# lukifer23/Matrix0

Measured on NVIDIA B200. Metric: MCTS sims/sec, batched self-play, ResNet-24 (BASELINE configs[3]), higher is better.
Workload: dtype fp16

## Files before the change

matrix0_b200/csrc/nn_attention_tc.cu:

```cuda
#include "nn.cuh"
#include <cuda_fp16.h>
#include <cstdlib>

namespace m0 {

template <bool FP16>
__device__ __forceinline__ void mma16816(float (&d)[4], const uint32_t (&a)[4], const uint32_t (&b)[2]) {
  if (FP16) {
    asm volatile("mma.sync.aligned.m16n8k16.row.col.f32.f16.f16.f32 {%0,%1,%2,%3}, {%4,%5,%6,%7}, {%8,%9}, {%0,%1,%2,%3};"
                 : "+f"(d[0]), "+f"(d[1]), "+f"(d[2]), "+f"(d[3])
                 : "r"(a[0]), "r"(a[1]), "r"(a[2]), "r"(a[3]), "r"(b[0]), "r"(b[1]));
  } else {
    asm volatile("mma.sync.aligned.m16n8k16.row.col.f32.bf16.bf16.f32 {%0,%1,%2,%3}, {%4,%5,%6,%7}, {%8,%9}, {%0,%1,%2,%3};"
                 : "+f"(d[0]), "+f"(d[1]), "+f"(d[2]), "+f"(d[3])
                 : "r"(a[0]), "r"(a[1]), "r"(a[2]), "r"(a[3]), "r"(b[0]), "r"(b[1]));
  }
}
template <bool FP16>
__device__ __forceinline__ uint32_t pack2(float lo, float hi) {
  if (FP16) {
    __half2 h = __floats2half2_rn(lo, hi);
    return *reinterpret_cast<uint32_t*>(&h);
  }
  __nv_bfloat162 h = __floats2bfloat162_rn(lo, hi);
// ... 277 lines not shown
  if (staged) {
    const int smem = 2 * 64 * BIAS_LD * (int)sizeof(float) + 8 * ATT_STAGE_BYTES;
    static unsigned long long granted = 0;
    int dev = 0;
    cudaGetDevice(&dev);
    if (dev >= 64 || !((granted >> dev) & 1ull)) {
      cudaError_t e = cudaFuncSetAttribute(attention_tc_staged_kernel<true>, cudaFuncAttributeMaxDynamicSharedMemorySize, smem);
      if (e == cudaSuccess) e = cudaFuncSetAttribute(attention_tc_staged_kernel<false>, cudaFuncAttributeMaxDynamicSharedMemorySize, smem);
      if (e != cudaSuccess) { m0_set_error("attention_tc: cannot reserve %d bytes of shared memory (%s)", smem, cudaGetErrorString(e)); return M0_ERR_CUDA; }
      if (dev < 64) granted |= 1ull << dev;
    }
    dim3 grid(heads, (B + 8 * bpw - 1) / (8 * bpw));
    if (nn_half_format()) attention_tc_staged_kernel<true><<<grid, 256, smem, s>>>((const uint16_t*)qkv_half, rel_bias, (uint16_t*)out_half, B, C, mix, bpw);
    else attention_tc_staged_kernel<false><<<grid, 256, smem, s>>>((const uint16_t*)qkv_half, rel_bias, (uint16_t*)out_half, B, C, mix, bpw);
    return m0_check_launch("attention_tc_staged");
  }
  const int per_block = 8 * ATT_BOARDS_PER_WARP;
  dim3 grid(heads, (B + per_block - 1) / per_block);
  if (nn_half_format()) attention_tc_kernel<true><<<grid, 256, 0, s>>>((const uint16_t*)qkv_half, rel_bias, (uint16_t*)out_half, B, C, mix);
  else attention_tc_kernel<false><<<grid, 256, 0, s>>>((const uint16_t*)qkv_half, rel_bias, (uint16_t*)out_half, B, C, mix);
  return m0_check_launch("attention_tc");
}

}
```

matrix0_b200/csrc/nn_tc_kernels.cu:

```cuda
#include "net_host.cuh"
#include "tc_gemm.cuh"
#include "tc_conv_pair.cuh"
#include <new>
#include <stdlib.h>
#include <string.h>
#include <stdio.h>
#include <string>
#include <utility>
#include <vector>

using namespace m0;

namespace m0 {
int nn_se_apply_gn(const __nv_bfloat16* conv_out, const float* gate, float* x, const float* gamma, const float* beta, __nv_bfloat16* a_out, int B,
                   int C, int act, cudaStream_t s);
int nn_planes_to_nhwc_half(const float* planes, __nv_bfloat16* out, int B, int P, cudaStream_t s);
int nn_se_hidden(const float* part, int splits, long long split_stride, const float* b1, __nv_bfloat16* hidden, int B, int hid, int ld, int act,
                 cudaStream_t s);
int nn_gn_act_res(const float* x, const float* gamma, const float* beta, const float* residual, long long residual_bstride, float* out,
                  __nv_bfloat16* out_half, int B, int C, int act, cudaStream_t s);
int nn_attention_tc(const void* qkv_half, const float* rel_bias, void* out_half, int B, int C, int heads, float mix, cudaStream_t s);
int nn_se_tail(const float* part, int splits, long long split_stride, int ld, const float* b1, const float* w2t, const float* b2, float* gate, int B,
               int C, int hid, int act, cudaStream_t s);
int nn_value_tail(const float* gate, const float* h, const float* w3, const float* b3, float* values, int B, int C, cudaStream_t s);
int nn_se_gate(const float* pool, const float* w1t, const float* b1, const float* w2t, const float* b2, float* gate, int B, int C, int hid, int act,
               cudaStream_t s);
}

namespace m0 {
__global__ void transpose_f32_kernel(const float* __restrict__ in, float* __restrict__ out, int rows, int cols) {
  int i = blockIdx.x * blockDim.x + threadIdx.x;
  if (i >= rows * cols) return;
  int r = i / cols, c = i % cols;
  out[c * rows + r] = in[i];
}
__global__ void se_fold_kernel(const float* __restrict__ conv_w, const float* __restrict__ w1, float* __restrict__ out, int C, int hid) {
  const int K = 12 * C;
  const int i = blockIdx.x * blockDim.x + threadIdx.x;
  if (i >= hid * K) return;
  const int u = i / K, k = i - u * K;
  const int ci = k % C, j = (k / C) % 6, hb = k / (6 * C);
  unsigned plus = 0, minus = 0;
  switch (j) {
    case 0: plus = 0x1FF; break;
// ... 84 lines not shown
struct TcWeight {
  __nv_bfloat16* w = nullptr;
  CUtensorMap map;
  CUtensorMap map_pair;
  bool pair = false;
  int n = 0, k = 0, n_part = 0, cluster = 1;
  int n_launch = 0;
};

int pick_cluster(int n_part) {
  static int forced = -1;
  if (forced < 0) {
    const char* e = getenv("M0_TC_CLUSTER");
    forced = e ? atoi(e) : 0;
  }
  int cs = forced > 0 ? forced : 2;
  while (cs > 1 && ((n_part / cs) % 8 != 0 || n_part % cs != 0)) cs >>= 1;
  return cs;
}

struct TcBlock {
  TcWeight conv1, conv2, qkv, proj;
  TcWeight se_fold, se_w2;
};

struct TcState {
  int sm_count = 148;
  int max_smem = 0;
  size_t smem_pair[9] = {0, 0, 0, 0, 0, 0, 0, 0, 0};
  size_t smem_gemm = 0;
  TcWeight pst, inter;
  std::vector<TcBlock> blocks;
  float *pool = nullptr, *se_hid = nullptr, *se_gate = nullptr;
  std::vector<float*> se_w1t, se_w2t;
  bool se_fused = false;
  int hid_pad = 0;
  __nv_bfloat16 *prims = nullptr, *se_hid_h = nullptr;
  float* se_part = nullptr;
  int se_splits = 1;
  size_t se_rows = 0;
  CUtensorMap prims_mat, se_hid_mat;
  __nv_bfloat16* planes_h = nullptr;
  __nv_bfloat16* qkv_h = nullptr;
  bool heads_tc = false;
  TcWeight pol_conv, pol_fc1, pol_fc2, val_conv1, val_conv2, val_fc1, val_fc2, val_gate;
  bool val_tail_tc = false;
  int pol_rank_pad = 0;
  __nv_bfloat16 *ph_h = nullptr, *pf_h = nullptr, *vh_h = nullptr;
  __nv_bfloat16 *vf1_h = nullptr, *vf2_h = nullptr;
  CUtensorMap ph_mat, pf_mat, vh_conv_mat, vh_fc_mat, vf1_mat, vf2_mat;
  CUtensorMap planes_conv;
  TcWeight stem;
  int cap = 0;
  __nv_bfloat16 *a1 = nullptr, *a2 = nullptr;
  CUtensorMap a1_conv, a2_conv, a1_mat, a2_mat;
  CUtensorMap a1_convp, a2_convp, planes_convp;
  CUtensorMap x_io;
  const void* x_ptr = nullptr;
  CUtensorMap qkv_out, t2f_out;
  CUtensorMap a1_out, a2_out, t1_out, t2h_out;
  const void *t1_ptr = nullptr, *t2_ptr = nullptr;
  int out_rows = 0;
  std::vector<void*> allocs;
};

// ... 300 lines not shown
  if (st->se_gate) cudaFree(st->se_gate);
  if (st->planes_h) cudaFree(st->planes_h);
  if (st->qkv_h) cudaFree(st->qkv_h);
  if (st->ph_h) cudaFree(st->ph_h);
  if (st->pf_h) cudaFree(st->pf_h);
  if (st->vh_h) cudaFree(st->vh_h);
  if (st->vf1_h) cudaFree(st->vf1_h);
  if (st->vf2_h) cudaFree(st->vf2_h);
  st->vf1_h = st->vf2_h = nullptr;
  if (st->prims) cudaFree(st->prims);
  if (st->se_hid_h) cudaFree(st->se_hid_h);
  if (st->se_part) cudaFree(st->se_part);
  st->se_part = nullptr;
  st->prims = st->se_hid_h = nullptr;
  st->qkv_h = st->ph_h = st->pf_h = st->vh_h = nullptr;
  st->a1 = st->a2 = nullptr;
  st->pool = st->se_hid = st->se_gate = nullptr;
  st->planes_h = nullptr;
  st->cap = 0;
  M0_CUDA_TRY(cudaMalloc((void**)&st->pool, (size_t)need * 2 * C * 4));
  M0_CUDA_TRY(cudaMalloc((void**)&st->se_hid, (size_t)need * (n->cfg.se_hidden > 0 ? n->cfg.se_hidden : 1) * 4));
  M0_CUDA_TRY(cudaMalloc((void**)&st->se_gate, (size_t)need * C * 4));
  M0_CUDA_TRY(cudaMalloc((void**)&st->planes_h, (size_t)need * 64 * 64 * 2));
  M0_CUDA_TRY(cudaMalloc((void**)&st->qkv_h, (size_t)need * 64 * 3 * C * 2));
  if (st->heads_tc) {
    const size_t rp = (size_t)st->pol_rank_pad;
    M0_CUDA_TRY(cudaMalloc((void**)&st->ph_h, (size_t)need * 4096 * 2));
    M0_CUDA_TRY(cudaMalloc((void**)&st->pf_h, (size_t)need * rp * 2));
    M0_CUDA_TRY(cudaMalloc((void**)&st->vh_h, (size_t)need * 8192 * 2));
    M0_CUDA_TRY(cudaMemset(st->pf_h, 0, (size_t)need * rp * 2));
    TRY(make_map_2d(&st->ph_mat, st->ph_h, (uint64_t)need, 4096, 128));
    TRY(make_map_2d(&st->pf_mat, st->pf_h, (uint64_t)need, rp, 128));
    TRY(make_map_2d(&st->vh_conv_mat, st->vh_h, (uint64_t)need * 64, 128, 128));
    TRY(make_map_2d(&st->vh_fc_mat, st->vh_h, (uint64_t)need, 8192, 128));
    if (st->val_tail_tc) {
      M0_CUDA_TRY(cudaMalloc((void**)&st->vf1_h, (size_t)need * 2 * C * 2));
      M0_CUDA_TRY(cudaMalloc((void**)&st->vf2_h, (size_t)need * C * 2));
      TRY(make_map_2d(&st->vf1_mat, st->vf1_h, (uint64_t)need, 2 * C, 128));
      TRY(make_map_2d(&st->vf2_mat, st->vf2_h, (uint64_t)need, C, 128));
    }
  }
  if (st->se_fused && n->cfg.se) {
    const size_t rows = ((size_t)need + 127) / 128 * 128;
    M0_CUDA_TRY(cudaMalloc((void**)&st->prims, rows * 12 * C * 2));
    M0_CUDA_TRY(cudaMalloc((void**)&st->se_hid_h, rows * st->hid_pad * 2));
    M0_CUDA_TRY(cudaMemset(st->prims, 0, rows * 12 * C * 2));
    M0_CUDA_TRY(cudaMemset(st->se_hid_h, 0, rows * st->hid_pad * 2));
// ... 77 lines not shown
      if ((rc = m0_check_cuda(cudaMemsetAsync(w2p, 0, (size_t)ps_pad * rp * 4, s), "memset")) != M0_OK) break;
      if ((rc = m0_check_cuda(cudaMemcpy2DAsync(w2p, (size_t)rp * 4, n->w.pol_fc2_w, (size_t)r * 4, (size_t)r * 4, c.policy_size,
                                                cudaMemcpyDeviceToDevice, s), "pad pol_fc2")) != M0_OK) break;
      if ((rc = make_weight(st, &st->pol_conv, n->w.pol_conv_w, 64, C, 64, s)) != M0_OK) break;
      if ((rc = make_weight(st, &st->pol_fc1, n->w.pol_fc1_w, r, 4096, r, s)) != M0_OK) break;
      if ((rc = make_weight(st, &st->pol_fc2, w2p, ps_pad, rp, 320, s)) != M0_OK) break;
      if ((rc = make_weight(st, &st->val_conv1, n->w.val_conv1_w, 128, C, 128, s)) != M0_OK) break;
      if ((rc = make_weight(st, &st->val_conv2, n->w.val_conv2_w, 128, 128, 128, s)) != M0_OK) break;
      const int fc1_launch = n_part_for(C) % 32 == 0 ? C : slice_width_for(C, C);
      if ((rc = make_weight(st, &st->val_fc1, n->w.val_fc1_w, 2 * C, 8192, fc1_launch, s)) != M0_OK) break;
      if (env_int("M0_TC_VALUE_TAIL", 1)) {
        if ((rc = make_weight(st, &st->val_fc2, n->w.val_fc2_w, C, 2 * C, slice_width_for(C, C), s)) != M0_OK) break;
        if ((rc = make_weight(st, &st->val_gate, n->w.val_gate_w, C, C, slice_width_for(C, C), s)) != M0_OK) break;
        st->val_tail_tc = true;
      }
      st->heads_tc = true;
    }
    if (c.chess_features) {
      if (c.piece_square_tables && (rc = make_weight(st, &st->pst, n->w.pst_w, C, C, env_int("M0_TC_SLICE_PROJ", 1) ? slice_width_for(C, C) : C, s)) != M0_OK) break;
      if ((rc = make_weight(st, &st->inter, n->w.inter_w, C, 9 * C, C, s, 9)) != M0_OK) break;
    }
    st->hid_pad = (c.se_hidden + 63) / 64 * 64;
    st->se_fused = env_int("M0_TC_FUSE_SE", 1) != 0 && pair_ok(C) && (!c.se || c.se_hidden <= 256);
    st->blocks.resize(c.blocks);
    for (int i = 0; i < c.blocks && rc == M0_OK; ++i) {
      const m0_block_weights& b = n->w.blocks[i];
      if ((rc = make_weight(st, &st->blocks[i].conv1, b.conv1_w, C, 9 * C, C, s, 9)) != M0_OK) break;
      if ((rc = make_weight(st, &st->blocks[i].conv2, b.conv2_w, C, 9 * C, C, s, 9)) != M0_OK) break;
      if (st->se_fused && c.se) {
        const int hid = c.se_hidden, hid16 = (hid + 15) / 16 * 16, K = 12 * C, hp = st->hid_pad;
        float *fold = nullptr, *w2p = nullptr;
        if ((rc = m0_check_cuda(cudaMalloc((void**)&fold, (size_t)hid16 * K * 4), "cudaMalloc se_fold")) != M0_OK) break;
        st->allocs.push_back(fold);
        if ((rc = m0_check_cuda(cudaMemsetAsync(fold, 0, (size_t)hid16 * K * 4, s), "memset se_fold")) != M0_OK) break;
        if ((rc = m0_check_cuda(cudaMalloc((void**)&w2p, (size_t)C * hp * 4), "cudaMalloc se_w2")) != M0_OK) break;
        st->allocs.push_back(w2p);
        se_fold_kernel<<<(hid * K + 255) / 256, 256, 0, s>>>(b.conv2_w, b.se_w1, fold, C, hid);
        pad_cols_kernel<float><<<(C * hp + 255) / 256, 256, 0, s>>>(b.se_w2, w2p, C, hid, hp);
        if ((rc = m0_check_launch("se_fold")) != M0_OK) break;
        if ((rc = make_weight(st, &st->blocks[i].se_fold, fold, hid16, K, hid16, s)) != M0_OK) break;
        if ((rc = make_weight(st, &st->blocks[i].se_w2, w2p, C, hp, C, s)) != M0_OK) break;
      }
      if (b.has_attention) {
        if ((rc = make_weight(st, &st->blocks[i].qkv, b.att_qkv_w, 3 * C, C, slice_width_for(3 * C, C), s)) != M0_OK) break;
        if ((rc = make_weight(st, &st->blocks[i].proj, b.att_proj_w, C, C, env_int("M0_TC_SLICE_PROJ", 1) ? slice_width_for(C, C) : C, s)) != M0_OK) break;
      }
    }
  } while (0);
  if (rc != M0_OK) {
    for (void* p : st->allocs) cudaFree(p);
    delete st;
    return rc;
  }
  all->st[fmt] = st;
  return M0_OK;
}

void tc_net_release(::m0_net* n) {
  TcStates* all = (TcStates*)n->tc;
  if (!all) return;
  for (int f = 0; f < 2; ++f) {
    TcState* st = all->st[f];
    if (!st) continue;
    for (void* p : st->allocs) cudaFree(p);
    if (st->a1) cudaFree(st->a1);
    if (st->a2) cudaFree(st->a2);
    if (st->pool) cudaFree(st->pool);
// ... 9 lines not shown
    if (st->prims) cudaFree(st->prims);
    if (st->se_hid_h) cudaFree(st->se_hid_h);
    if (st->se_part) cudaFree(st->se_part);
    delete st;
  }
  delete all;
  n->tc = nullptr;
}

int tc_net_forward(::m0_net* n, const float* planes, int B, float* logits, float* values, cudaStream_t s) {
  TcState* st = ((TcStates*)n->tc)->st[nn_half_format()];
  TRY(net_ws_reserve(n, B));
  TRY(tc_reserve(n, st, B));
  const m0_net_config& c = n->cfg;
  const m0_net_weights& w = n->w;
  const int C = c.channels, M = B * 64, act = c.activation;
  const float* none = nullptr;
  if (st->t1_ptr != n->t1 || st->t2_ptr != n->t2 || st->x_ptr != n->x || st->out_rows != M) {
    TRY(make_map_out(&st->a1_out, st->a1, (uint64_t)M, C, false));
    TRY(make_map_out(&st->a2_out, st->a2, (uint64_t)M, C, false));
    TRY(make_map_out(&st->t1_out, n->t1, (uint64_t)M, C, true));
    TRY(make_map_out(&st->t2h_out, n->t2, (uint64_t)M, C, false));
    TRY(make_map_out(&st->t2f_out, n->t2, (uint64_t)M, C, true));
    TRY(make_map_out(&st->qkv_out, st->qkv_h, (uint64_t)M, 3 * (uint64_t)C, false));
    TRY(make_map_out(&st->x_io, n->x, (uint64_t)M, C, true, true));
    st->x_ptr = n->x;
    st->t1_ptr = n->t1;
    st->t2_ptr = n->t2;
    st->out_rows = M;
  }
  PROF("planes_to_nhwc_half", nn_planes_to_nhwc_half(planes, st->planes_h, B, c.planes, s));
  PROF("conv_other", conv3x3(st, st->planes_conv, st->planes_convp, st->stem, B, 64, n->t1, nullptr, ACT_NONE, s, nullptr, nullptr, nullptr, nullptr, &st->t1_out));
  if (c.chess_features) {
    PROF("gn_act_res", nn_gn_act_res(n->t1, w.stem_gn_w, w.stem_gn_b, w.pos_enc, 0, n->x, st->a1, B, C, act, s));
    float* cur = n->x;
    if (c.piece_square_tables) {
      PROF("gemm_pst", gemm_rows64(st, st->a1_mat, st->pst, B, C, n->t1, nullptr, C, s, &st->t1_out));
      PROF("gn_act_res", nn_gn_act_res(n->t1, w.pst_gn_w, w.pst_gn_b, n->x, (long long)64 * C, n->t2, st->a1, B, C, act, s));
      cur = n->t2;
    }
    PROF("conv_other", conv3x3(st, st->a1_conv, st->a1_convp, st->inter, B, C, n->t1, nullptr, ACT_NONE, s, nullptr, nullptr, nullptr, nullptr, &st->t1_out));
    PROF("gn_act_res", nn_gn_act_res(n->t1, w.inter_gn_w, w.inter_gn_b, cur, (long long)64 * C, n->x, nullptr, B, C, act, s));
  } else {
    PROF("groupnorm_f32", nn_groupnorm_f32(n->t1, w.stem_gn_w, w.stem_gn_b, nullptr, 0, n->x, B, C, act, s));
  }
  if (c.blocks > 0) PROF("se_apply_gn", nn_se_apply_gn(nullptr, nullptr, n->x, w.blocks[0].gn1_w, w.blocks[0].gn1_b, st->a1, B, C, act, s));
  int att_seen = 0;
// ... 37 lines not shown
      se_done:;
      }
      ConvFusion f2;
      f2.resid_x = n->x;
      f2.gate = c.se ? st->se_gate : nullptr;
      f2.x_map = &st->x_io;
      PROF("conv2+se+res+gn", conv3x3(st, st->a2_conv, st->a2_convp, tb.conv2, B, C, nullptr, next_a, act, s, fuse_next ? w.blocks[i + 1].gn1_w : nullptr,
                                      fuse_next ? w.blocks[i + 1].gn1_b : nullptr, nullptr, &f2, next_a ? &st->a1_out : nullptr));
    } else {
      PROF("conv1+gn", conv3x3(st, st->a1_conv, st->a1_convp, tb.conv1, B, C, nullptr, st->a2, act, s, b.gn2_w, b.gn2_b, nullptr, nullptr, &st->a2_out));
      __nv_bfloat16* t2h = reinterpret_cast<__nv_bfloat16*>(n->t2);
      PROF("conv2+pool", conv3x3(st, st->a2_conv, st->a2_convp, tb.conv2, B, C, nullptr, t2h, ACT_NONE, s, nullptr, nullptr, c.se ? st->pool : nullptr, nullptr,
                                 &st->t2h_out));
      const float* gate = nullptr;
      if (c.se) {
        PROF("se_gate", nn_se_gate(st->pool, st->se_w1t[i], b.se_b1, st->se_w2t[i], b.se_b2, st->se_gate, B, C, c.se_hidden, act, s));
        gate = st->se_gate;
      }
      PROF("se_apply_gn", nn_se_apply_gn(t2h, gate, n->x, fuse_next ? w.blocks[i + 1].gn1_w : nullptr, fuse_next ? w.blocks[i + 1].gn1_b : nullptr,
                                         next_a, B, C, act, s));
    }
    if (run_att) {
      const float* rb = c.attention_relbias ? b.att_rel_bias : nullptr;
      if (tc_att) {
        PROF("gemm_qkv", gemm_rows64(st, st->a1_mat, tb.qkv, B, C, nullptr, st->qkv_h, 3 * C, s, &st->qkv_out));
        PROF("attention_tc", nn_attention_tc(st->qkv_h, rb, st->a2, B, C, c.attention_heads, c.attention_unmasked_mix, s));
      } else {
        PROF("gemm_qkv", gemm_rows64(st, st->a1_mat, tb.qkv, B, C, n->qkv, nullptr, 3 * C, s));
        PROF("attention_f32", nn_attention_f32(n->qkv, rb, n->t1, B, C, c.attention_heads, c.attention_unmasked_mix, s));
        PROF("f32_to_bf16", nn_f32_to_bf16(n->t1, st->a2, (size_t)M * C, s));
      }
      static int proj_f32 = -1;
      if (proj_f32 < 0) proj_f32 = env_int("M0_TC_PROJ_F32", 0);
      const bool fused_ln = C % 32 == 0 && C <= 320;
      const bool proj_half = fused_ln && !proj_f32;
      if (proj_half) PROF("gemm_proj", gemm_rows64(st, st->a2_mat, tb.proj, B, C, nullptr, reinterpret_cast<__nv_bfloat16*>(n->t2), C, s, &st->t2h_out));
      else PROF("gemm_proj", gemm_rows64(st, st->a2_mat, tb.proj, B, C, n->t2, nullptr, C, s, &st->t2f_out));
      if (fused_ln) {
        heads_input_ready = last && st->heads_tc;
        PROF("ln_res_gn", nn_ln_res_gn(n->t2, proj_half ? 1 : 0, n->x, b.att_ln_w, b.att_ln_b, last ? nullptr : w.blocks[i + 1].gn1_w,
                                       last ? nullptr : w.blocks[i + 1].gn1_b, (last && !st->heads_tc) ? nullptr : st->a1, B, C, act, s));
      } else {
        PROF("layernorm_residual_f32", nn_layernorm_residual_f32(n->t2, n->x, b.att_ln_w, b.att_ln_b, n->x, M, C, s));
        if (!last) PROF("se_apply_gn", nn_se_apply_gn(nullptr, nullptr, n->x, w.blocks[i + 1].gn1_w, w.blocks[i + 1].gn1_b, st->a1, B, C, act, s));
      }
    }
  }
// ... 116 lines not shown
```

matrix0_b200/csrc/tc_gemm.cuh:

```cuda
#pragma once
#include <cuda.h>
#include <cuda_bf16.h>
#include <cuda_fp16.h>
#include "nn.cuh"

namespace m0 {
namespace tc {

static constexpr int BM = 128;
static constexpr int BK = 64;
static constexpr int A_TILE_BYTES = BM * BK * 2;
static constexpr int NUM_THREADS = 320;

__device__ __forceinline__ uint32_t smem_u32(const void* p) { return (uint32_t)__cvta_generic_to_shared(p); }

__device__ __forceinline__ void mbar_init(uint64_t* bar, uint32_t count) {
  asm volatile("mbarrier.init.shared::cta.b64 [%0], %1;" ::"r"(smem_u32(bar)), "r"(count) : "memory");
}
__device__ __forceinline__ void mbar_expect_tx(uint64_t* bar, uint32_t bytes) {
  asm volatile("mbarrier.arrive.expect_tx.shared::cta.b64 _, [%0], %1;" ::"r"(smem_u32(bar)), "r"(bytes) : "memory");
}
__device__ __forceinline__ void mbar_arrive(uint64_t* bar) {
  asm volatile("mbarrier.arrive.shared::cta.b64 _, [%0];" ::"r"(smem_u32(bar)) : "memory");
}
__device__ __forceinline__ void mbar_wait(uint64_t* bar, uint32_t parity) {
  asm volatile(
      "{\n\t"
      ".reg .pred p;\n\t"
      "WAIT_%=:\n\t"
      "mbarrier.try_wait.parity.shared::cta.b64 p, [%0], %1;\n\t"
      "@p bra DONE_%=;\n\t"
      "bra WAIT_%=;\n\t"
      "DONE_%=:\n\t"
      "}\n" ::"r"(smem_u32(bar)), "r"(parity)
      : "memory");
}
__device__ __forceinline__ void fence_barrier_init() { asm volatile("fence.mbarrier_init.release.cluster;" ::: "memory"); }
__device__ __forceinline__ void fence_proxy_async() { asm volatile("fence.proxy.async.shared::cta;" ::: "memory"); }

__device__ __forceinline__ void tma_prefetch_desc(const CUtensorMap* m) {
  asm volatile("prefetch.tensormap [%0];" ::"l"(reinterpret_cast<uint64_t>(m)) : "memory");
}
__device__ __forceinline__ void tma_load_2d(void* dst, const CUtensorMap* map, uint64_t* bar, int c0, int c1) {
  asm volatile("cp.async.bulk.tensor.2d.shared::cluster.global.mbarrier::complete_tx::bytes [%0], [%1, {%3, %4}], [%2];" ::"r"(smem_u32(dst)),
               "l"(reinterpret_cast<uint64_t>(map)), "r"(smem_u32(bar)), "r"(c0), "r"(c1)
               : "memory");
}
__device__ __forceinline__ void tma_load_4d(void* dst, const CUtensorMap* map, uint64_t* bar, int c0, int c1, int c2, int c3) {
  asm volatile("cp.async.bulk.tensor.4d.shared::cluster.global.mbarrier::complete_tx::bytes [%0], [%1, {%3, %4, %5, %6}], [%2];" ::"r"(
                   smem_u32(dst)),
               "l"(reinterpret_cast<uint64_t>(map)), "r"(smem_u32(bar)), "r"(c0), "r"(c1), "r"(c2), "r"(c3)
               : "memory");
}

__device__ __forceinline__ void tma_load_2d_mcast(void* dst, const CUtensorMap* map, uint64_t* bar, int c0, int c1, uint16_t cta_mask) {
  asm volatile(
      "cp.async.bulk.tensor.2d.shared::cluster.global.mbarrier::complete_tx::bytes.multicast::cluster [%0], [%1, {%3, %4}], [%2], %5;" ::"r"(
          smem_u32(dst)),
      "l"(reinterpret_cast<uint64_t>(map)), "r"(smem_u32(bar)), "r"(c0), "r"(c1), "h"(cta_mask)
      : "memory");
}
__device__ __forceinline__ bool elect_one() {
  uint32_t pred;
  asm volatile(
      "{\n\t"
      ".reg .pred P;\n\t"
      "elect.sync _|P, 0xFFFFFFFF;\n\t"
      "selp.u32 %0, 1, 0, P;\n\t"
      "}\n"
      : "=r"(pred));
  return pred != 0;
}
__device__ __forceinline__ uint32_t cluster_ctarank() {
  uint32_t r;
  asm volatile("mov.u32 %0, %%cluster_ctarank;" : "=r"(r));
  return r;
}
__device__ __forceinline__ void cluster_sync_all() {
  asm volatile("barrier.cluster.arrive.release.aligned;" ::: "memory");
  asm volatile("barrier.cluster.wait.acquire.aligned;" ::: "memory");
}

__device__ __forceinline__ void tmem_alloc(uint32_t* dst_smem, uint32_t cols) {
  asm volatile("tcgen05.alloc.cta_group::1.sync.aligned.shared::cta.b32 [%0], %1;" ::"r"(smem_u32(dst_smem)), "r"(cols) : "memory");
}
__device__ __forceinline__ void tmem_relinquish() { asm volatile("tcgen05.relinquish_alloc_permit.cta_group::1.sync.aligned;" ::: "memory"); }
__device__ __forceinline__ void tmem_dealloc(uint32_t addr, uint32_t cols) {
  asm volatile("tcgen05.dealloc.cta_group::1.sync.aligned.b32 %0, %1;" ::"r"(addr), "r"(cols) : "memory");
}
__device__ __forceinline__ void tc_fence_before() { asm volatile("tcgen05.fence::before_thread_sync;" ::: "memory"); }
__device__ __forceinline__ void tc_fence_after() { asm volatile("tcgen05.fence::after_thread_sync;" ::: "memory"); }

__device__ __forceinline__ void umma_bf16(uint32_t tmem_d, uint64_t desc_a, uint64_t desc_b, uint32_t idesc, uint32_t accumulate) {
  asm volatile(
      "{\n\t"
      ".reg .pred p;\n\t"
      "setp.ne.b32 p, %4, 0;\n\t"
      "tcgen05.mma.cta_group::1.kind::f16 [%0], %1, %2, %3, p;\n\t"
      "}\n" ::"r"(tmem_d),
      "l"(desc_a), "l"(desc_b), "r"(idesc), "r"(accumulate)
      : "memory");
}
__device__ __forceinline__ void umma_commit(uint64_t* bar) {
  asm volatile("tcgen05.commit.cta_group::1.mbarrier::arrive::one.shared::cluster.b64 [%0];" ::"r"(smem_u32(bar)) : "memory");
}
__device__ __forceinline__ void umma_commit_mcast(uint64_t* bar, uint16_t cta_mask) {
  asm volatile("tcgen05.commit.cta_group::1.mbarrier::arrive::one.shared::cluster.multicast::cluster.b64 [%0], %1;" ::"r"(smem_u32(bar)),
               "h"(cta_mask)
               : "memory");
}
__device__ __forceinline__ void tmem_ld_32x32(uint32_t taddr, uint32_t (&r)[32]) {
  asm volatile(
      "tcgen05.ld.sync.aligned.32x32b.x32.b32 "
      "{%0, %1, %2, %3, %4, %5, %6, %7, %8, %9, %10, %11, %12, %13, %14, %15, "
      "%16, %17, %18, %19, %20, %21, %22, %23, %24, %25, %26, %27, %28, %29, %30, %31}, [%32];"
      : "=r"(r[0]), "=r"(r[1]), "=r"(r[2]), "=r"(r[3]), "=r"(r[4]), "=r"(r[5]), "=r"(r[6]), "=r"(r[7]), "=r"(r[8]), "=r"(r[9]), "=r"(r[10]),
        "=r"(r[11]), "=r"(r[12]), "=r"(r[13]), "=r"(r[14]), "=r"(r[15]), "=r"(r[16]), "=r"(r[17]), "=r"(r[18]), "=r"(r[19]), "=r"(r[20]),
        "=r"(r[21]), "=r"(r[22]), "=r"(r[23]), "=r"(r[24]), "=r"(r[25]), "=r"(r[26]), "=r"(r[27]), "=r"(r[28]), "=r"(r[29]), "=r"(r[30]),
        "=r"(r[31])
      : "r"(taddr));
}
__device__ __forceinline__ void tmem_ld_wait() { asm volatile("tcgen05.wait::ld.sync.aligned;" ::: "memory"); }

__device__ __forceinline__ uint64_t make_smem_desc(uint32_t smem_addr) {
  return (uint64_t)((smem_addr >> 4) & 0x3FFFu) | (1ull << 16) | (64ull << 32) | (1ull << 46) | (2ull << 61);
}
__host__ __device__ __forceinline__ uint32_t make_idesc_bf16(int m, int n, int fp16 = 0) {
  const uint32_t fmt = fp16 ? 0u : 1u;
  return (1u << 4) | (fmt << 7) | (fmt << 10) | ((uint32_t)(n >> 3) << 17) | ((uint32_t)(m >> 4) << 24);
}

struct GemmParams {
  int M;
  int N;
  int n_store;
  int n_part;
  int taps;
  int kb_per_tap;
  int conv;
  int w_row0;
  int stages;
  int tmem_cols;
  int fp16;
  int cluster;
  float* out_f32;
  __nv_bfloat16* out_bf16;
  int ldc, col0;
  const float* bias;
  int act;
  float scale;
  const float* gn_gamma;
  const float* gn_beta;
  float* pool_part;
// ... 304 lines not shown
```

Measured before the change: 13.92 million.

## Fuse QKV projection GEMM into tcgen05 attention kernel with TMEM-staged per-head tiles

Adds a persistent warp-specialized kernel in which one warp issues TMA loads of activations and per-head QKV weight slices, one warp issues tcgen05 MMAs into a multi-buffered TMEM accumulator, and three consumer groups drain TMEM into shared memory and run the existing mma.sync attention per head pair. This removes the separate QKV GEMM launch and the global round trip through the qkv_h buffer, which is no longer allocated by default. In exchange, QKV weights are re-read per head group, the kernel carries heavy shared-memory and TMEM requirements, and it is limited to head_dim 16, even head counts and C<=320.

```diff
diff --git a/matrix0_b200/csrc/nn_attention_tc.cu b/matrix0_b200/csrc/nn_attention_tc.cu
--- a/matrix0_b200/csrc/nn_attention_tc.cu
+++ b/matrix0_b200/csrc/nn_attention_tc.cu
@@ -1,4 +1,5 @@
 #include "nn.cuh"
+#include "tc_ptx.cuh"
 #include <cuda_fp16.h>
 #include <cstdlib>
 
@@ -323,4 +324,220 @@
   return m0_check_launch("attention_tc");
 }
 
-}
+namespace fused {
+constexpr int HPC = 2;
+constexpr int NQKV = 48 * HPC;
+constexpr int NG = 3;
+constexpr int STAGES = 3;
+constexpr int NACC = 4;
+constexpr int A_BYTES = 128 * 64 * 2;
+constexpr int STAGE_BYTES = A_BYTES + NQKV * 128;
+constexpr int GROUP_BYTES = 2 * HPC * ATT_STAGE_BYTES;
+constexpr int THREADS = 64 + NG * 128;
+constexpr int SMEM = STAGES * STAGE_BYTES + NG * GROUP_BYTES + (HPC + 1) * 64 * BIAS_LD * 4 + 256 + 1024;
+}
+
+template <bool FP16>
+__global__ void __launch_bounds__(fused::THREADS, 1)
+attention_fused_kernel(const __grid_constant__ CUtensorMap tma_a, const __grid_constant__ CUtensorMap tma_w, const float* __restrict__ rel_bias,
+                       uint16_t* __restrict__ out, int B, int C, int head_groups, float mix) {
+  using namespace fused;
+  using namespace tc;
+  extern __shared__ __align__(1024) uint8_t fused_smem_raw[];
+  uint8_t* smem = fused_smem_raw + ((1024u - (smem_u32(fused_smem_raw) & 1023u)) & 1023u);
+  uint8_t* qkv_stage = smem + STAGES * STAGE_BYTES;
+  float* s_bias = reinterpret_cast<float*>(qkv_stage + NG * GROUP_BYTES);
+  float* s_mask = s_bias + HPC * 64 * BIAS_LD;
+  uint64_t* full_bar = reinterpret_cast<uint64_t*>(s_mask + 64 * BIAS_LD);
+  uint64_t* empty_bar = full_bar + STAGES;
+  uint64_t* tmem_full = empty_bar + STAGES;
+  uint64_t* tmem_empty = tmem_full + NACC;
+  uint32_t* tmem_slot = reinterpret_cast<uint32_t*>(tmem_empty + NACC);
+
+  const int warp = threadIdx.x >> 5, lane = threadIdx.x & 31;
+  const int hg = blockIdx.x % head_groups, walker = blockIdx.x / head_groups, walkers = gridDim.x / head_groups;
+  const int tiles = (B + 1) >> 1, kblocks = (C + 63) >> 6;
+
+  if (warp == 0 && lane == 0) {
+    tma_prefetch_desc(&tma_a);
+    tma_prefetch_desc(&tma_w);
+    for (int s = 0; s < STAGES; ++s) { mbar_init(&full_bar[s], 1); mbar_init(&empty_bar[s], 1); }
+    for (int a = 0; a < NACC; ++a) { mbar_init(&tmem_full[a], 1); mbar_init(&tmem_empty[a], 128); }
+    fence_barrier_init();
+  }
+  if (warp == 1) {
+    tmem_alloc(tmem_slot, 512);
+    tmem_relinquish();
+  }
+  for (int i = threadIdx.x; i < 64 * 64; i += THREADS) {
+    const int o = (i >> 6) * BIAS_LD + (i & 63);
+#pragma unroll
+    for (int hh = 0; hh < HPC; ++hh)
+      s_bias[hh * 64 * BIAS_LD + o] = rel_bias ? rel_bias[(size_t)(hg * HPC + hh) * 4096 + i] * LOG2E : 0.0f;
+    s_mask[o] = attn_mask_tc(i >> 6, i & 63) ? 1.0f : 0.0f;
+  }
+  tc_fence_before();
+  __syncthreads();
+  tc_fence_after();
+
+  if (warp == 0) {
+    if (lane == 0) {
+      int stage = 0;
+      uint32_t phase = 0;
+      for (int j = walker; j < tiles; j += walkers)
+        for (int kb = 0; kb < kblocks; ++kb) {
+          mbar_wait(&empty_bar[stage], phase ^ 1);
+          uint8_t* dst = smem + stage * STAGE_BYTES;
+          mbar_expect_tx(&full_bar[stage], (uint32_t)STAGE_BYTES);
+          tma_load_2d(dst, &tma_a, &full_bar[stage], kb * 64, j * 128);
+#pragma unroll
+          for (int p = 0; p < 3 * HPC; ++p)
+            tma_load_2d(dst + A_BYTES + p * 16 * 128, &tma_w, &full_bar[stage], kb * 64, (p % 3) * C + (hg * HPC + p / 3) * 16);
+          if (++stage == STAGES) { stage = 0; phase ^= 1; }
+        }
+    }
+  } else if (warp == 1) {
+    const uint32_t tmem_base = *tmem_slot;
+    const uint32_t idesc = make_idesc_bf16(128, NQKV, FP16 ? 1 : 0);
+    const uint32_t smem_base = smem_u32(smem);
+    int stage = 0;
+    uint32_t phase = 0, it = 0;
+    for (int j = walker; j < tiles; j += walkers, ++it) {
+      const uint32_t acc = it % NACC, acc_phase = (it / NACC) & 1u;
+      mbar_wait(&tmem_empty[acc], acc_phase ^ 1);
+      tc_fence_after();
+      const uint32_t tmem_acc = tmem_base + acc * 128;
+      for (int kb = 0; kb < kblocks; ++kb) {
+        mbar_wait(&full_bar[stage], phase);
+        tc_fence_after();
+        const uint32_t a_addr = smem_base + (uint32_t)(stage * STAGE_BYTES);
+        const uint64_t adesc = make_smem_desc(a_addr), bdesc = make_smem_desc(a_addr + A_BYTES);
+        if (elect_one()) {
+#pragma unroll
+          for (int k = 0; k < 4; ++k) umma_bf16(tmem_acc, adesc + 2 * k, bdesc + 2 * k, idesc, (kb > 0 || k > 0) ? 1u : 0u);
+          umma_commit(&empty_bar[stage]);
+        }
+        __syncwarp();
+        if (++stage == STAGES) { stage = 0; phase ^= 1; }
+      }
+      if (elect_one()) umma_commit(&tmem_full[acc]);
+      __syncwarp();
+    }
+  } else {
+    asm volatile("st.shared.u32 [%0], %1;" ::"r"(smem_u32(tmem_slot + 1 + warp)), "r"((uint32_t)(warp - 2) >> 2) : "memory");
+#pragma unroll 1
+    for (;;) {
+      uint32_t tid, cta, ncta, it;
+      asm volatile("mov.u32 %0, %%tid.x;" : "=r"(tid));
+      asm volatile("ld.shared.u32 %0, [%1];" : "=r"(it) : "r"(smem_u32(tmem_slot + 1 + (tid >> 5))) : "memory");
+      asm volatile("mov.u32 %0, %%ctaid.x;" : "=r"(cta));
+      asm volatile("mov.u32 %0, %%nctaid.x;" : "=r"(ncta));
+      const int j = (int)(cta / head_groups) + (int)it * (int)(ncta / head_groups);
+      if (j >= tiles) break;
+      const int grp = ((int)(tid >> 5) - 2) >> 2, quarter = (tid >> 5) & 3, ln = tid & 31;
+      uint8_t* gbuf = qkv_stage + grp * GROUP_BYTES;
+      uint8_t* row_dst = gbuf + (quarter >> 1) * HPC * ATT_STAGE_BYTES + ((quarter & 1) * 32 + ln) * 32;
+      const uint32_t bar_id = 1 + grp;
+      uint32_t tmem_base_it;
+      asm volatile("ld.shared.u32 %0, [%1];" : "=r"(tmem_base_it) : "r"(smem_u32(tmem_slot)));
+      const uint32_t acc = it % NACC, acc_phase = (it / NACC) & 1u;
+      mbar_wait(&tmem_full[acc], acc_phase);
+      tc_fence_after();
+      const uint32_t trow = tmem_base_it + acc * 128 + ((uint32_t)(quarter * 32) << 16);
+#pragma unroll
+      for (int c = 0; c < NQKV / 32; ++c) {
+        uint32_t r[32];
+        tmem_ld_32x32(trow + 32 * c, r);
+        tmem_ld_wait();
+#pragma unroll
+        for (int hp = 0; hp < 2; ++hp) {
+          const int piece = 2 * c + hp;
+          uint4* dst = reinterpret_cast<uint4*>(row_dst + (piece / 3) * ATT_STAGE_BYTES + (piece % 3) * 2048);
+          uint32_t wv[8];
+#pragma unroll
+          for (int e = 0; e < 8; ++e) wv[e] = pack2<FP16>(__uint_as_float(r[16 * hp + 2 * e]), __uint_as_float(r[16 * hp + 2 * e + 1]));
+          dst[0] = make_uint4(wv[0], wv[1], wv[2], wv[3]);
+          dst[1] = make_uint4(wv[4], wv[5], wv[6], wv[7]);
+        }
+      }
+      tc_fence_before();
+      mbar_arrive(&tmem_empty[acc]);
+      asm volatile("bar.sync %0, 128;" ::"r"(bar_id) : "memory");
+      const int unit = quarter;
+      const uint16_t* sq = reinterpret_cast<const uint16_t*>(gbuf + unit * ATT_STAGE_BYTES), * sk = sq + 64 * 16, * sv = sq + 2 * 64 * 16;
+      const int g = ln >> 2, t = ln & 3;
+      uint32_t kf[8][2];
+#pragma unroll
+      for (int nt = 0; nt < 8; ++nt) {
+        const uint16_t* kr = sk + (8 * nt + g) * 16;
+        kf[nt][0] = *reinterpret_cast<const uint32_t*>(kr + 2 * t);
+        kf[nt][1] = *reinterpret_cast<const uint32_t*>(kr + 2 * t + 8);
+      }
+      uint32_t vf[4][2][2];
+#pragma unroll
+      for (int kk = 0; kk < 4; ++kk)
+#pragma unroll
+        for (int nd = 0; nd < 2; ++nd) {
+          const uint32_t lo = *reinterpret_cast<const uint32_t*>(sv + (16 * kk + g) * 16 + 8 * nd + 2 * t);
+          const uint32_t hi = *reinterpret_cast<const uint32_t*>(sv + (16 * kk + 8 + g) * 16 + 8 * nd + 2 * t);
+          vf[kk][nd][0] = movmatrix_trans(lo);
+          vf[kk][nd][1] = movmatrix_trans(hi);
+        }
+      uint32_t qall[4][4];
+#pragma unroll
+      for (int mt = 0; mt < 4; ++mt) {
+        const uint16_t* qr = sq + (16 * mt + g) * 16 + 2 * t;
+        qall[mt][0] = *reinterpret_cast<const uint32_t*>(qr);
+        qall[mt][1] = *reinterpret_cast<const uint32_t*>(qr + 8 * 16);
+        qall[mt][2] = *reinterpret_cast<const uint32_t*>(qr + 8);
+        qall[mt][3] = *reinterpret_cast<const uint32_t*>(qr + 8 * 16 + 8);
+      }
+      asm volatile("bar.sync %0, 128;" ::"r"(bar_id) : "memory");
+      asm volatile("st.shared.u32 [%0], %1;" ::"r"(smem_u32(tmem_slot + 1 + (tid >> 5))), "r"(it + NG) : "memory");
+      const int b = 2 * j + (unit >> 1);
+      if (b < B)
+        attend_head<FP16>(kf, vf, qall, s_bias + (unit & 1) * 64 * BIAS_LD, s_mask, out, b, (int)(cta % head_groups) * HPC + (unit & 1), C, g, t, mix);
+    }
+  }
+  tc_fence_before();
+  __syncthreads();
+  if (warp == 1) {
+    tc_fence_after();
+    tmem_dealloc(*tmem_slot, 512);
+  }
+}
+
+int nn_attention_fused(const CUtensorMap* a_map, const CUtensorMap* w_map, const float* rel_bias, void* out_half, int B, int C, int heads, float mix,
+                       cudaStream_t s) {
+  if (C != heads * 16 || heads % fused::HPC != 0 || C % 32 != 0 || C > 320) {
+    m0_set_error("attention_fused: needs head_dim 16, an even head count and C %% 32 == 0, C <= 320 (C=%d heads=%d)", C, heads);
+    return M0_ERR_ARG;
+  }
+  static unsigned long long granted = 0;
+  static int sms[64] = {0};
+  int dev = 0;
+  cudaGetDevice(&dev);
+  if (dev >= 64 || !((granted >> dev) & 1ull)) {
+    cudaError_t e = cudaFuncSetAttribute(attention_fused_kernel<true>, cudaFuncAttributeMaxDynamicSharedMemorySize, fused::SMEM);
+    if (e == cudaSuccess) e = cudaFuncSetAttribute(attention_fused_kernel<false>, cudaFuncAttributeMaxDynamicSharedMemorySize, fused::SMEM);
+    if (e != cudaSuccess) { m0_set_error("attention_fused: cannot reserve %d bytes of shared memory (%s)", fused::SMEM, cudaGetErrorString(e)); return M0_ERR_CUDA; }
+    if (dev < 64) {
+      cudaDeviceGetAttribute(&sms[dev], cudaDevAttrMultiProcessorCount, dev);
+      granted |= 1ull << dev;
+    }
+  }
+  int sm_count = 148;
+  if (dev < 64 && sms[dev] > 0) sm_count = sms[dev];
+  const int head_groups = heads / fused::HPC, tiles = (B + 1) / 2;
+  int walkers = sm_count / head_groups;
+  if (walkers < 1) walkers = 1;
+  if (walkers > tiles) walkers = tiles;
+  const dim3 grid((unsigned)(head_groups * walkers));
+  if (nn_half_format())
+    attention_fused_kernel<true><<<grid, fused::THREADS, fused::SMEM, s>>>(*a_map, *w_map, rel_bias, (uint16_t*)out_half, B, C, head_groups, mix);
+  else
+    attention_fused_kernel<false><<<grid, fused::THREADS, fused::SMEM, s>>>(*a_map, *w_map, rel_bias, (uint16_t*)out_half, B, C, head_groups, mix);
+  return m0_check_launch("attention_fused");
+}
+
+}
diff --git a/matrix0_b200/csrc/nn_tc_kernels.cu b/matrix0_b200/csrc/nn_tc_kernels.cu
--- a/matrix0_b200/csrc/nn_tc_kernels.cu
+++ b/matrix0_b200/csrc/nn_tc_kernels.cu
@@ -20,6 +20,8 @@
 int nn_gn_act_res(const float* x, const float* gamma, const float* beta, const float* residual, long long residual_bstride, float* out,
                   __nv_bfloat16* out_half, int B, int C, int act, cudaStream_t s);
 int nn_attention_tc(const void* qkv_half, const float* rel_bias, void* out_half, int B, int C, int heads, float mix, cudaStream_t s);
+int nn_attention_fused(const CUtensorMap* a_map, const CUtensorMap* w_map, const float* rel_bias, void* out_half, int B, int C, int heads, float mix,
+                       cudaStream_t s);
 int nn_se_tail(const float* part, int splits, long long split_stride, int ld, const float* b1, const float* w2t, const float* b2, float* gate, int B,
                int C, int hid, int act, cudaStream_t s);
 int nn_value_tail(const float* gate, const float* h, const float* w3, const float* b3, float* values, int B, int C, cudaStream_t s);
@@ -150,6 +152,7 @@
 struct TcBlock {
   TcWeight conv1, conv2, qkv, proj;
   TcWeight se_fold, se_w2;
+  CUtensorMap qkv_heads;
 };
 
 struct TcState {
@@ -169,6 +172,7 @@
   size_t se_rows = 0;
   CUtensorMap prims_mat, se_hid_mat;
   __nv_bfloat16* planes_h = nullptr;
+  bool att_fused = true;
   __nv_bfloat16* qkv_h = nullptr;
   bool heads_tc = false;
   TcWeight pol_conv, pol_fc1, pol_fc2, val_conv1, val_conv2, val_fc1, val_fc2, val_gate;
@@ -515,7 +519,7 @@
   M0_CUDA_TRY(cudaMalloc((void**)&st->se_hid, (size_t)need * (n->cfg.se_hidden > 0 ? n->cfg.se_hidden : 1) * 4));
   M0_CUDA_TRY(cudaMalloc((void**)&st->se_gate, (size_t)need * C * 4));
   M0_CUDA_TRY(cudaMalloc((void**)&st->planes_h, (size_t)need * 64 * 64 * 2));
-  M0_CUDA_TRY(cudaMalloc((void**)&st->qkv_h, (size_t)need * 64 * 3 * C * 2));
+  if (!st->att_fused) M0_CUDA_TRY(cudaMalloc((void**)&st->qkv_h, (size_t)need * 64 * 3 * C * 2));
   if (st->heads_tc) {
     const size_t rp = (size_t)st->pol_rank_pad;
     M0_CUDA_TRY(cudaMalloc((void**)&st->ph_h, (size_t)need * 4096 * 2));
@@ -639,6 +643,7 @@
     }
     st->hid_pad = (c.se_hidden + 63) / 64 * 64;
     st->se_fused = env_int("M0_TC_FUSE_SE", 1) != 0 && pair_ok(C) && (!c.se || c.se_hidden <= 256);
+    st->att_fused = env_int("M0_ATT_FUSED", 1) != 0;
     st->blocks.resize(c.blocks);
     for (int i = 0; i < c.blocks && rc == M0_OK; ++i) {
       const m0_block_weights& b = n->w.blocks[i];
@@ -660,6 +665,7 @@
       }
       if (b.has_attention) {
         if ((rc = make_weight(st, &st->blocks[i].qkv, b.att_qkv_w, 3 * C, C, slice_width_for(3 * C, C), s)) != M0_OK) break;
+        if (st->att_fused && (rc = make_map_2d(&st->blocks[i].qkv_heads, st->blocks[i].qkv.w, 3 * (uint64_t)C, (uint64_t)C, 16)) != M0_OK) break;
         if ((rc = make_weight(st, &st->blocks[i].proj, b.att_proj_w, C, C, env_int("M0_TC_SLICE_PROJ", 1) ? slice_width_for(C, C) : C, s)) != M0_OK) break;
       }
     }
@@ -715,7 +721,7 @@
     TRY(make_map_out(&st->t1_out, n->t1, (uint64_t)M, C, true));
     TRY(make_map_out(&st->t2h_out, n->t2, (uint64_t)M, C, false));
     TRY(make_map_out(&st->t2f_out, n->t2, (uint64_t)M, C, true));
-    TRY(make_map_out(&st->qkv_out, st->qkv_h, (uint64_t)M, 3 * (uint64_t)C, false));
+    if (st->qkv_h) TRY(make_map_out(&st->qkv_out, st->qkv_h, (uint64_t)M, 3 * (uint64_t)C, false));
     TRY(make_map_out(&st->x_io, n->x, (uint64_t)M, C, true, true));
     st->x_ptr = n->x;
     st->t1_ptr = n->t1;
@@ -799,7 +805,9 @@
     }
     if (run_att) {
       const float* rb = c.attention_relbias ? b.att_rel_bias : nullptr;
-      if (tc_att) {
+      if (tc_att && st->att_fused) {
+        PROF("attention_tc", nn_attention_fused(&st->a1_mat, &tb.qkv_heads, rb, st->a2, B, C, c.attention_heads, c.attention_unmasked_mix, s));
+      } else if (tc_att) {
         PROF("gemm_qkv", gemm_rows64(st, st->a1_mat, tb.qkv, B, C, nullptr, st->qkv_h, 3 * C, s, &st->qkv_out));
         PROF("attention_tc", nn_attention_tc(st->qkv_h, rb, st->a2, B, C, c.attention_heads, c.attention_unmasked_mix, s));
       } else {
diff --git a/matrix0_b200/csrc/tc_gemm.cuh b/matrix0_b200/csrc/tc_gemm.cuh
--- a/matrix0_b200/csrc/tc_gemm.cuh
+++ b/matrix0_b200/csrc/tc_gemm.cuh
@@ -3,6 +3,7 @@
 #include <cuda_bf16.h>
 #include <cuda_fp16.h>
 #include "nn.cuh"
+#include "tc_ptx.cuh"
 
 namespace m0 {
 namespace tc {
@@ -11,124 +12,6 @@
 static constexpr int BK = 64;
 static constexpr int A_TILE_BYTES = BM * BK * 2;
 static constexpr int NUM_THREADS = 320;
-
-__device__ __forceinline__ uint32_t smem_u32(const void* p) { return (uint32_t)__cvta_generic_to_shared(p); }
-
-__device__ __forceinline__ void mbar_init(uint64_t* bar, uint32_t count) {
-  asm volatile("mbarrier.init.shared::cta.b64 [%0], %1;" ::"r"(smem_u32(bar)), "r"(count) : "memory");
-}
-__device__ __forceinline__ void mbar_expect_tx(uint64_t* bar, uint32_t bytes) {
-  asm volatile("mbarrier.arrive.expect_tx.shared::cta.b64 _, [%0], %1;" ::"r"(smem_u32(bar)), "r"(bytes) : "memory");
-}
-__device__ __forceinline__ void mbar_arrive(uint64_t* bar) {
-  asm volatile("mbarrier.arrive.shared::cta.b64 _, [%0];" ::"r"(smem_u32(bar)) : "memory");
-}
-__device__ __forceinline__ void mbar_wait(uint64_t* bar, uint32_t parity) {
-  asm volatile(
-      "{\n\t"
-      ".reg .pred p;\n\t"
-      "WAIT_%=:\n\t"
-      "mbarrier.try_wait.parity.shared::cta.b64 p, [%0], %1;\n\t"
-      "@p bra DONE_%=;\n\t"
-      "bra WAIT_%=;\n\t"
-      "DONE_%=:\n\t"
-      "}\n" ::"r"(smem_u32(bar)), "r"(parity)
-      : "memory");
-}
-__device__ __forceinline__ void fence_barrier_init() { asm volatile("fence.mbarrier_init.release.cluster;" ::: "memory"); }
-__device__ __forceinline__ void fence_proxy_async() { asm volatile("fence.proxy.async.shared::cta;" ::: "memory"); }
-
-__device__ __forceinline__ void tma_prefetch_desc(const CUtensorMap* m) {
-  asm volatile("prefetch.tensormap [%0];" ::"l"(reinterpret_cast<uint64_t>(m)) : "memory");
-}
-__device__ __forceinline__ void tma_load_2d(void* dst, const CUtensorMap* map, uint64_t* bar, int c0, int c1) {
-  asm volatile("cp.async.bulk.tensor.2d.shared::cluster.global.mbarrier::complete_tx::bytes [%0], [%1, {%3, %4}], [%2];" ::"r"(smem_u32(dst)),
-               "l"(reinterpret_cast<uint64_t>(map)), "r"(smem_u32(bar)), "r"(c0), "r"(c1)
-               : "memory");
-}
-__device__ __forceinline__ void tma_load_4d(void* dst, const CUtensorMap* map, uint64_t* bar, int c0, int c1, int c2, int c3) {
-  asm volatile("cp.async.bulk.tensor.4d.shared::cluster.global.mbarrier::complete_tx::bytes [%0], [%1, {%3, %4, %5, %6}], [%2];" ::"r"(
-                   smem_u32(dst)),
-               "l"(reinterpret_cast<uint64_t>(map)), "r"(smem_u32(bar)), "r"(c0), "r"(c1), "r"(c2), "r"(c3)
-               : "memory");
-}
-
-__device__ __forceinline__ void tma_load_2d_mcast(void* dst, const CUtensorMap* map, uint64_t* bar, int c0, int c1, uint16_t cta_mask) {
-  asm volatile(
-      "cp.async.bulk.tensor.2d.shared::cluster.global.mbarrier::complete_tx::bytes.multicast::cluster [%0], [%1, {%3, %4}], [%2], %5;" ::"r"(
-          smem_u32(dst)),
-      "l"(reinterpret_cast<uint64_t>(map)), "r"(smem_u32(bar)), "r"(c0), "r"(c1), "h"(cta_mask)
-      : "memory");
-}
-__device__ __forceinline__ bool elect_one() {
-  uint32_t pred;
-  asm volatile(
-      "{\n\t"
-      ".reg .pred P;\n\t"
-      "elect.sync _|P, 0xFFFFFFFF;\n\t"
-      "selp.u32 %0, 1, 0, P;\n\t"
-      "}\n"
-      : "=r"(pred));
-  return pred != 0;
-}
-__device__ __forceinline__ uint32_t cluster_ctarank() {
-  uint32_t r;
-  asm volatile("mov.u32 %0, %%cluster_ctarank;" : "=r"(r));
-  return r;
-}
-__device__ __forceinline__ void cluster_sync_all() {
-  asm volatile("barrier.cluster.arrive.release.aligned;" ::: "memory");
-  asm volatile("barrier.cluster.wait.acquire.aligned;" ::: "memory");
-}
-
-__device__ __forceinline__ void tmem_alloc(uint32_t* dst_smem, uint32_t cols) {
-  asm volatile("tcgen05.alloc.cta_group::1.sync.aligned.shared::cta.b32 [%0], %1;" ::"r"(smem_u32(dst_smem)), "r"(cols) : "memory");
-}
-__device__ __forceinline__ void tmem_relinquish() { asm volatile("tcgen05.relinquish_alloc_permit.cta_group::1.sync.aligned;" ::: "memory"); }
-__device__ __forceinline__ void tmem_dealloc(uint32_t addr, uint32_t cols) {
-  asm volatile("tcgen05.dealloc.cta_group::1.sync.aligned.b32 %0, %1;" ::"r"(addr), "r"(cols) : "memory");
-}
-__device__ __forceinline__ void tc_fence_before() { asm volatile("tcgen05.fence::before_thread_sync;" ::: "memory"); }
-__device__ __forceinline__ void tc_fence_after() { asm volatile("tcgen05.fence::after_thread_sync;" ::: "memory"); }
-
-__device__ __forceinline__ void umma_bf16(uint32_t tmem_d, uint64_t desc_a, uint64_t desc_b, uint32_t idesc, uint32_t accumulate) {
-  asm volatile(
-      "{\n\t"
-      ".reg .pred p;\n\t"
-      "setp.ne.b32 p, %4, 0;\n\t"
-      "tcgen05.mma.cta_group::1.kind::f16 [%0], %1, %2, %3, p;\n\t"
-      "}\n" ::"r"(tmem_d),
-      "l"(desc_a), "l"(desc_b), "r"(idesc), "r"(accumulate)
-      : "memory");
-}
-__device__ __forceinline__ void umma_commit(uint64_t* bar) {
-  asm volatile("tcgen05.commit.cta_group::1.mbarrier::arrive::one.shared::cluster.b64 [%0];" ::"r"(smem_u32(bar)) : "memory");
-}
-__device__ __forceinline__ void umma_commit_mcast(uint64_t* bar, uint16_t cta_mask) {
-  asm volatile("tcgen05.commit.cta_group::1.mbarrier::arrive::one.shared::cluster.multicast::cluster.b64 [%0], %1;" ::"r"(smem_u32(bar)),
-               "h"(cta_mask)
-               : "memory");
-}
-__device__ __forceinline__ void tmem_ld_32x32(uint32_t taddr, uint32_t (&r)[32]) {
-  asm volatile(
-      "tcgen05.ld.sync.aligned.32x32b.x32.b32 "
-      "{%0, %1, %2, %3, %4, %5, %6, %7, %8, %9, %10, %11, %12, %13, %14, %15, "
-      "%16, %17, %18, %19, %20, %21, %22, %23, %24, %25, %26, %27, %28, %29, %30, %31}, [%32];"
-      : "=r"(r[0]), "=r"(r[1]), "=r"(r[2]), "=r"(r[3]), "=r"(r[4]), "=r"(r[5]), "=r"(r[6]), "=r"(r[7]), "=r"(r[8]), "=r"(r[9]), "=r"(r[10]),
-        "=r"(r[11]), "=r"(r[12]), "=r"(r[13]), "=r"(r[14]), "=r"(r[15]), "=r"(r[16]), "=r"(r[17]), "=r"(r[18]), "=r"(r[19]), "=r"(r[20]),
-        "=r"(r[21]), "=r"(r[22]), "=r"(r[23]), "=r"(r[24]), "=r"(r[25]), "=r"(r[26]), "=r"(r[27]), "=r"(r[28]), "=r"(r[29]), "=r"(r[30]),
-        "=r"(r[31])
-      : "r"(taddr));
-}
-__device__ __forceinline__ void tmem_ld_wait() { asm volatile("tcgen05.wait::ld.sync.aligned;" ::: "memory"); }
-
-__device__ __forceinline__ uint64_t make_smem_desc(uint32_t smem_addr) {
-  return (uint64_t)((smem_addr >> 4) & 0x3FFFu) | (1ull << 16) | (64ull << 32) | (1ull << 46) | (2ull << 61);
-}
-__host__ __device__ __forceinline__ uint32_t make_idesc_bf16(int m, int n, int fp16 = 0) {
-  const uint32_t fmt = fp16 ? 0u : 1u;
-  return (1u << 4) | (fmt << 7) | (fmt << 10) | ((uint32_t)(n >> 3) << 17) | ((uint32_t)(m >> 4) << 24);
-}
 
 struct GemmParams {
   int M;
diff --git a/matrix0_b200/csrc/tc_ptx.cuh b/matrix0_b200/csrc/tc_ptx.cuh
--- /dev/null
+++ b/matrix0_b200/csrc/tc_ptx.cuh
@@ -0,0 +1,127 @@
+#pragma once
+#include <cuda.h>
+#include <cstdint>
+
+namespace m0 {
+namespace tc {
+
+__device__ __forceinline__ uint32_t smem_u32(const void* p) { return (uint32_t)__cvta_generic_to_shared(p); }
+
+__device__ __forceinline__ void mbar_init(uint64_t* bar, uint32_t count) {
+  asm volatile("mbarrier.init.shared::cta.b64 [%0], %1;" ::"r"(smem_u32(bar)), "r"(count) : "memory");
+}
+__device__ __forceinline__ void mbar_expect_tx(uint64_t* bar, uint32_t bytes) {
+  asm volatile("mbarrier.arrive.expect_tx.shared::cta.b64 _, [%0], %1;" ::"r"(smem_u32(bar)), "r"(bytes) : "memory");
+}
+__device__ __forceinline__ void mbar_arrive(uint64_t* bar) {
+  asm volatile("mbarrier.arrive.shared::cta.b64 _, [%0];" ::"r"(smem_u32(bar)) : "memory");
+}
+__device__ __forceinline__ void mbar_wait(uint64_t* bar, uint32_t parity) {
+  asm volatile(
+      "{\n\t"
+      ".reg .pred p;\n\t"
+      "WAIT_%=:\n\t"
+      "mbarrier.try_wait.parity.shared::cta.b64 p, [%0], %1;\n\t"
+      "@p bra DONE_%=;\n\t"
+      "bra WAIT_%=;\n\t"
+      "DONE_%=:\n\t"
+      "}\n" ::"r"(smem_u32(bar)), "r"(parity)
+      : "memory");
+}
+__device__ __forceinline__ void fence_barrier_init() { asm volatile("fence.mbarrier_init.release.cluster;" ::: "memory"); }
+__device__ __forceinline__ void fence_proxy_async() { asm volatile("fence.proxy.async.shared::cta;" ::: "memory"); }
+
+__device__ __forceinline__ void tma_prefetch_desc(const CUtensorMap* m) {
+  asm volatile("prefetch.tensormap [%0];" ::"l"(reinterpret_cast<uint64_t>(m)) : "memory");
+}
+__device__ __forceinline__ void tma_load_2d(void* dst, const CUtensorMap* map, uint64_t* bar, int c0, int c1) {
+  asm volatile("cp.async.bulk.tensor.2d.shared::cluster.global.mbarrier::complete_tx::bytes [%0], [%1, {%3, %4}], [%2];" ::"r"(smem_u32(dst)),
+               "l"(reinterpret_cast<uint64_t>(map)), "r"(smem_u32(bar)), "r"(c0), "r"(c1)
+               : "memory");
+}
+__device__ __forceinline__ void tma_load_4d(void* dst, const CUtensorMap* map, uint64_t* bar, int c0, int c1, int c2, int c3) {
+  asm volatile("cp.async.bulk.tensor.4d.shared::cluster.global.mbarrier::complete_tx::bytes [%0], [%1, {%3, %4, %5, %6}], [%2];" ::"r"(
+                   smem_u32(dst)),
+               "l"(reinterpret_cast<uint64_t>(map)), "r"(smem_u32(bar)), "r"(c0), "r"(c1), "r"(c2), "r"(c3)
+               : "memory");
+}
+
+__device__ __forceinline__ void tma_load_2d_mcast(void* dst, const CUtensorMap* map, uint64_t* bar, int c0, int c1, uint16_t cta_mask) {
+  asm volatile(
+      "cp.async.bulk.tensor.2d.shared::cluster.global.mbarrier::complete_tx::bytes.multicast::cluster [%0], [%1, {%3, %4}], [%2], %5;" ::"r"(
+          smem_u32(dst)),
+      "l"(reinterpret_cast<uint64_t>(map)), "r"(smem_u32(bar)), "r"(c0), "r"(c1), "h"(cta_mask)
+      : "memory");
+}
+__device__ __forceinline__ bool elect_one() {
+  uint32_t pred;
+  asm volatile(
+      "{\n\t"
+      ".reg .pred P;\n\t"
+      "elect.sync _|P, 0xFFFFFFFF;\n\t"
+      "selp.u32 %0, 1, 0, P;\n\t"
+      "}\n"
+      : "=r"(pred));
+  return pred != 0;
+}
+__device__ __forceinline__ uint32_t cluster_ctarank() {
+  uint32_t r;
+  asm volatile("mov.u32 %0, %%cluster_ctarank;" : "=r"(r));
+  return r;
+}
+__device__ __forceinline__ void cluster_sync_all() {
+  asm volatile("barrier.cluster.arrive.release.aligned;" ::: "memory");
+  asm volatile("barrier.cluster.wait.acquire.aligned;" ::: "memory");
+}
+
+__device__ __forceinline__ void tmem_alloc(uint32_t* dst_smem, uint32_t cols) {
+  asm volatile("tcgen05.alloc.cta_group::1.sync.aligned.shared::cta.b32 [%0], %1;" ::"r"(smem_u32(dst_smem)), "r"(cols) : "memory");
+}
+__device__ __forceinline__ void tmem_relinquish() { asm volatile("tcgen05.relinquish_alloc_permit.cta_group::1.sync.aligned;" ::: "memory"); }
+__device__ __forceinline__ void tmem_dealloc(uint32_t addr, uint32_t cols) {
+  asm volatile("tcgen05.dealloc.cta_group::1.sync.aligned.b32 %0, %1;" ::"r"(addr), "r"(cols) : "memory");
+}
+__device__ __forceinline__ void tc_fence_before() { asm volatile("tcgen05.fence::before_thread_sync;" ::: "memory"); }
+__device__ __forceinline__ void tc_fence_after() { asm volatile("tcgen05.fence::after_thread_sync;" ::: "memory"); }
+
+__device__ __forceinline__ void umma_bf16(uint32_t tmem_d, uint64_t desc_a, uint64_t desc_b, uint32_t idesc, uint32_t accumulate) {
+  asm volatile(
+      "{\n\t"
+      ".reg .pred p;\n\t"
+      "setp.ne.b32 p, %4, 0;\n\t"
+      "tcgen05.mma.cta_group::1.kind::f16 [%0], %1, %2, %3, p;\n\t"
+      "}\n" ::"r"(tmem_d),
+      "l"(desc_a), "l"(desc_b), "r"(idesc), "r"(accumulate)
+      : "memory");
+}
+__device__ __forceinline__ void umma_commit(uint64_t* bar) {
+  asm volatile("tcgen05.commit.cta_group::1.mbarrier::arrive::one.shared::cluster.b64 [%0];" ::"r"(smem_u32(bar)) : "memory");
+}
+__device__ __forceinline__ void umma_commit_mcast(uint64_t* bar, uint16_t cta_mask) {
+  asm volatile("tcgen05.commit.cta_group::1.mbarrier::arrive::one.shared::cluster.multicast::cluster.b64 [%0], %1;" ::"r"(smem_u32(bar)),
+               "h"(cta_mask)
+               : "memory");
+}
+__device__ __forceinline__ void tmem_ld_32x32(uint32_t taddr, uint32_t (&r)[32]) {
+  asm volatile(
+      "tcgen05.ld.sync.aligned.32x32b.x32.b32 "
+      "{%0, %1, %2, %3, %4, %5, %6, %7, %8, %9, %10, %11, %12, %13, %14, %15, "
+      "%16, %17, %18, %19, %20, %21, %22, %23, %24, %25, %26, %27, %28, %29, %30, %31}, [%32];"
+      : "=r"(r[0]), "=r"(r[1]), "=r"(r[2]), "=r"(r[3]), "=r"(r[4]), "=r"(r[5]), "=r"(r[6]), "=r"(r[7]), "=r"(r[8]), "=r"(r[9]), "=r"(r[10]),
+        "=r"(r[11]), "=r"(r[12]), "=r"(r[13]), "=r"(r[14]), "=r"(r[15]), "=r"(r[16]), "=r"(r[17]), "=r"(r[18]), "=r"(r[19]), "=r"(r[20]),
+        "=r"(r[21]), "=r"(r[22]), "=r"(r[23]), "=r"(r[24]), "=r"(r[25]), "=r"(r[26]), "=r"(r[27]), "=r"(r[28]), "=r"(r[29]), "=r"(r[30]),
+        "=r"(r[31])
+      : "r"(taddr));
+}
+__device__ __forceinline__ void tmem_ld_wait() { asm volatile("tcgen05.wait::ld.sync.aligned;" ::: "memory"); }
+
+__device__ __forceinline__ uint64_t make_smem_desc(uint32_t smem_addr) {
+  return (uint64_t)((smem_addr >> 4) & 0x3FFFu) | (1ull << 16) | (64ull << 32) | (1ull << 46) | (2ull << 61);
+}
+__host__ __device__ __forceinline__ uint32_t make_idesc_bf16(int m, int n, int fp16 = 0) {
+  const uint32_t fmt = fp16 ? 0u : 1u;
+  return (1u << 4) | (fmt << 7) | (fmt << 10) | ((uint32_t)(n >> 3) << 17) | ((uint32_t)(m >> 4) << 24);
+}
+
+}
+}
```

New measurement: 14.18 million, median of 6. +1.9%, better.
